# thrill/thrill

Measured on AMD Instinct MI355X. Metric: TeraSort keys/sec (100-byte recs), higher is better.
Workload: dtype u8; 1 GPU; terasort_10GiB_100B; records=107374182, record_bytes=100, seed=0x7421, parallelism=dp1

## Files before the change

thrill_amd/csrc/t9_sort_msb9.hip:

```cpp

#include "t9_common.h"
#include "t9_rank_scatter.h"

#include <cstdlib>
#include <vector>

#define T9_MSB_TILE 8192
#define NDIG9 512

__device__ inline u32 bucket_of9(const u32* s_abase, u32 pos) {
    u32 lo = 0, hi = 255;
    while (lo < hi) {
        u32 mid = (lo + hi + 1) >> 1;
        if (s_abase[mid] <= pos) lo = mid; else hi = mid - 1;
    }
    return lo;
}

__global__ __launch_bounds__(256) void k_hist_seg9(
    const u64* __restrict__ keys, const u32* __restrict__ abase,
    const u32* __restrict__ bucket_n, u32* __restrict__ hist) {
    __shared__ u32 s_cnt[NDIG9];
    __shared__ u32 s_abase[257];
    const u32 tid = threadIdx.x;
    s_abase[tid] = abase[tid];
    if (tid == 0) s_abase[256] = abase[256];
    s_cnt[tid] = 0;
    s_cnt[tid + 256] = 0;
    __syncthreads();
    const u64 tbase64 = (u64)blockIdx.x * T9_MSB_TILE;
    if (tbase64 < s_abase[256]) {
        const u32 tbase = (u32)tbase64;
        const u32 b = bucket_of9(s_abase, tbase);
        const u32 off = tbase - s_abase[b];
        const u32 tn = (bucket_n[b] > off)
                           ? ((bucket_n[b] - off < T9_MSB_TILE)
                                  ? bucket_n[b] - off
                                  : T9_MSB_TILE)
                           : 0;
        const u32 lane = tid & 63;
        for (u32 i0 = 0; i0 < (u32)T9_MSB_TILE; i0 += 256) {
            const u32 i = i0 + tid;
            const bool valid = i < tn;
            const u32 d =
                valid ? (u32)(keys[tbase + i] >> 47) & 511u : 0;
            t9_hist_ballot_add<9>(s_cnt, d, valid, lane);
        }
    }
    __syncthreads();
    hist[(u64)blockIdx.x * NDIG9 + tid] = s_cnt[tid];
    hist[(u64)blockIdx.x * NDIG9 + tid + 256] = s_cnt[tid + 256];
}

__global__ __launch_bounds__(256) void k_seg_scan9(
    u32* __restrict__ hist, const u32* __restrict__ abase,
    const u32* __restrict__ bucket_n, const u32* __restrict__ true_base,
    u32* __restrict__ sub_start, u32* __restrict__ sub_n) {
    const u32 b = blockIdx.x;
    const u32 tid = threadIdx.x;
    const u32 r0 = abase[b] / T9_MSB_TILE;
    const u32 rows = (bucket_n[b] + T9_MSB_TILE - 1) / T9_MSB_TILE;
    u32 tot0 = 0, tot1 = 0;
    for (u32 r = 0; r < rows; ++r) {
        tot0 += hist[(u64)(r0 + r) * NDIG9 + tid];
        tot1 += hist[(u64)(r0 + r) * NDIG9 + tid + 256];
    }
    __shared__ u32 sh[NDIG9];
    sh[tid] = tot0;
    sh[tid + 256] = tot1;
    __syncthreads();
    t9_scan_onewave<NDIG9>(sh, tid);
    __syncthreads();
    const u32 gstart0 = true_base[b] + sh[tid];
    const u32 gstart1 = true_base[b] + sh[tid + 256];
    sub_start[(u64)b * NDIG9 + tid] = gstart0;
    sub_start[(u64)b * NDIG9 + tid + 256] = gstart1;
    sub_n[(u64)b * NDIG9 + tid] = tot0;
    sub_n[(u64)b * NDIG9 + tid + 256] = tot1;
    u32 run0 = gstart0, run1 = gstart1;
    for (u32 r = 0; r < rows; ++r) {
        u32 v0 = hist[(u64)(r0 + r) * NDIG9 + tid];
        u32 v1 = hist[(u64)(r0 + r) * NDIG9 + tid + 256];
        hist[(u64)(r0 + r) * NDIG9 + tid] = run0;
        hist[(u64)(r0 + r) * NDIG9 + tid + 256] = run1;
        run0 += v0;
        run1 += v1;
    }
}

template <bool HAS_VAL>
__global__ __launch_bounds__(1024, 4) void k_scatter_seg9(
    const u64* __restrict__ in_keys, const u32* __restrict__ in_vals,
    const u32* __restrict__ abase, const u32* __restrict__ bucket_n,
    u64* __restrict__ out_keys, u32* __restrict__ out_vals,
    const u32* __restrict__ offs) {
    constexpr int TILE = T9_MSB_TILE;
    constexpr int NW = 16;
    constexpr int SUB = TILE / NW;
    constexpr int GROUPS = SUB / 64;
    __shared__ u64 s_okeys[TILE];
    __shared__ u32 s_ovals[HAS_VAL ? TILE : 1];
    __shared__ u16 s_rank[TILE];
    __shared__ u16 s_wcnt[NW * NDIG9];
    __shared__ u16 s_woff[NW * NDIG9];
    __shared__ u32 s_start[NDIG9];
    __shared__ u32 s_goff[NDIG9];
    __shared__ u32 s_abase[257];

    const u32 tid = threadIdx.x, wave = tid >> 6, lane = tid & 63;
    if (tid < 257) s_abase[tid] = abase[tid];
    __syncthreads();
    const u64 tbase64 = (u64)blockIdx.x * TILE;
    if (tbase64 >= s_abase[256]) return;
    const u32 tbase = (u32)tbase64;
    const u32 b = bucket_of9(s_abase, tbase);
    const u32 off_in_bucket = tbase - s_abase[b];
    const u32 bn = bucket_n[b];
    const u32 tn = (bn > off_in_bucket)
                       ? ((bn - off_in_bucket < (u32)TILE)
                              ? bn - off_in_bucket
                              : (u32)TILE)
                       : 0;

    if (tid < NDIG9)
        s_goff[tid] = offs[(u64)blockIdx.x * NDIG9 + tid];
    for (u32 t = lane; t < NDIG9; t += 64) s_wcnt[wave * NDIG9 + t] = 0;

    const u32 wbase = wave * SUB;
    for (int g = 0; g < GROUPS; ++g) {
        const u32 i = wbase + g * 64 + lane;
        const bool valid = i < tn;
        u32 d = 0;
        if (valid) d = (u32)(in_keys[tbase + i] >> 47) & 511u;
        u64 m = __ballot(valid);
        for (int bit = 0; bit < 9; ++bit) {
            u64 bb = __ballot((d >> bit) & 1u);
            m &= ((d >> bit) & 1u) ? bb : ~bb;
        }
        const u32 wr = (u32)__popcll(m & ((1ull << lane) - 1ull));
        const u32 before = valid ? (u32)s_wcnt[wave * NDIG9 + d] : 0;
        if (valid) {
            s_rank[i] = (u16)(before + wr);
            if (wr == 0)
                s_wcnt[wave * NDIG9 + d] =
                    (u16)(before + (u32)__popcll(m));
        }
    }
    __syncthreads();

    if (tid < NDIG9) {
        u32 run = 0;
        for (int w = 0; w < NW; ++w) {
            s_woff[w * NDIG9 + tid] = (u16)run;
            run += s_wcnt[w * NDIG9 + tid];
        }
        s_start[tid] = run;
    }
    __syncthreads();
    t9_scan_onewave<NDIG9>(s_start, tid);
    __syncthreads();

    for (int g = 0; g < GROUPS; ++g) {
        const u32 i = wbase + g * 64 + lane;
        if (i < tn) {
            const u64 k = in_keys[tbase + i];
            const u32 d = (u32)(k >> 47) & 511u;
            const u32 pos = s_start[d] + (u32)s_woff[wave * NDIG9 + d] +
                            s_rank[i];
            s_okeys[pos] = k;
            if (HAS_VAL) s_ovals[pos] = in_vals[tbase + i];
        }
    }
    __syncthreads();

    constexpr int CHUNKS = TILE / 1024;
    for (int c = 0; c < CHUNKS; ++c) {
        const u32 j = c * 1024 + tid;
        if (j < tn) {
            const u32 d = (u32)(s_okeys[j] >> 47) & 511u;
            const u64 gpos = (u64)s_goff[d] + (j - s_start[d]);
            out_keys[gpos] = s_okeys[j];
            if (HAS_VAL) out_vals[gpos] = s_ovals[j];
        }
    }
}

extern "C" {

void t9i_launch_hist_seg9(u32 grid, void* stream, const u64* keys,
                          const u32* abase, const u32* bucket_n,
                          u32* hist) {
    hipLaunchKernelGGL(k_hist_seg9, dim3(grid), dim3(256), 0,
                       (hipStream_t)stream, keys, abase, bucket_n, hist);
}

void t9i_launch_seg_scan9(u32 grid, void* stream, u32* hist,
                          const u32* abase, const u32* bucket_n,
                          const u32* true_base, u32* sub_start,
                          u32* sub_n) {
    hipLaunchKernelGGL(k_seg_scan9, dim3(grid), dim3(256), 0,
                       (hipStream_t)stream, hist, abase, bucket_n,
                       true_base, sub_start, sub_n);
}

void t9i_launch_scatter_seg9(u32 grid, int has_val, void* stream,
                             const u64* in_keys, const u32* in_vals,
                             const u32* abase, const u32* bucket_n,
                             u64* out_keys, u32* out_vals,
                             const u32* offs) {
    if (has_val)
        hipLaunchKernelGGL((k_scatter_seg9<true>), dim3(grid), dim3(1024),
                           0, (hipStream_t)stream, in_keys, in_vals, abase,
                           bucket_n, out_keys, out_vals, offs);
    else
        hipLaunchKernelGGL((k_scatter_seg9<false>), dim3(grid), dim3(1024),
                           0, (hipStream_t)stream, in_keys, in_vals, abase,
                           bucket_n, out_keys, out_vals, offs);
}

}
```

Baseline: 8.578 billion keys/s.

## Restructure MSB scatter kernel to cut LDS use and keep keys in registers

Rewrites the segmented 9-bit MSB scatter kernel. Keys and values are held in registers instead of being reloaded. The key and value staging buffers share one LDS region, per-key ranks are packed into registers, and the bucket lookup uses wave ballots instead of a shared-memory binary search. The digit scan uses shuffles, and tile indices are remapped so contiguous tiles land on the same XCD. The launch-bounds hint is raised so more blocks fit per CU. The risks are higher register pressure, which could cause spills at the new occupancy target, and subtle correctness hazards from aliasing LDS buffers and from the unconditional key loads past tn.

```diff
diff --git a/thrill_amd/csrc/t9_sort_msb9.hip b/thrill_amd/csrc/t9_sort_msb9.hip
--- a/thrill_amd/csrc/t9_sort_msb9.hip
+++ b/thrill_amd/csrc/t9_sort_msb9.hip
@@ -89,7 +89,7 @@
 }
 
 template <bool HAS_VAL>
-__global__ __launch_bounds__(1024, 4) void k_scatter_seg9(
+__global__ __launch_bounds__(1024, 8) void k_scatter_seg9(
     const u64* __restrict__ in_keys, const u32* __restrict__ in_vals,
     const u32* __restrict__ abase, const u32* __restrict__ bucket_n,
     u64* __restrict__ out_keys, u32* __restrict__ out_vals,
@@ -98,90 +98,162 @@
     constexpr int NW = 16;
     constexpr int SUB = TILE / NW;
     constexpr int GROUPS = SUB / 64;
-    __shared__ u64 s_okeys[TILE];
-    __shared__ u32 s_ovals[HAS_VAL ? TILE : 1];
-    __shared__ u16 s_rank[TILE];
-    __shared__ u16 s_wcnt[NW * NDIG9];
-    __shared__ u16 s_woff[NW * NDIG9];
-    __shared__ u32 s_start[NDIG9];
-    __shared__ u32 s_goff[NDIG9];
-    __shared__ u32 s_abase[257];
+    __shared__ __align__(16) u8 s_raw[TILE * 8];
+    u64* const s_okeys = (u64*)s_raw;
+    u32* const s_ovals = (u32*)s_raw;
+    static_assert(SUB <= 65535 && TILE <= 65535, "u16 counts and offsets");
+    static_assert(NW * 64 == 1024 && NDIG9 == 8 * 64,
+                  "one thread per key column, waves 0..7 own the digits");
+    __shared__ __align__(16) u16 s_wcnt[NW * NDIG9];
+    u32* const s_wtot = (u32*)s_raw;
+    u32* const s_delta = (u32*)s_wcnt;
 
     const u32 tid = threadIdx.x, wave = tid >> 6, lane = tid & 63;
-    if (tid < 257) s_abase[tid] = abase[tid];
-    __syncthreads();
-    const u64 tbase64 = (u64)blockIdx.x * TILE;
-    if (tbase64 >= s_abase[256]) return;
+    const u32 xper = gridDim.x >> 3, xrem = gridDim.x & 7;
+    const u32 xcd = blockIdx.x & 7;
+    const u32 tile = xcd * xper + (xcd < xrem ? xcd : xrem) +
+                     (blockIdx.x >> 3);
+    const u64 tbase64 = (u64)tile * TILE;
+    if (tbase64 >= abase[256]) return;
     const u32 tbase = (u32)tbase64;
-    const u32 b = bucket_of9(s_abase, tbase);
-    const u32 off_in_bucket = tbase - s_abase[b];
-    const u32 bn = bucket_n[b];
+
+    const u32 wbase = wave * SUB;
+    u64 key[GROUPS];
+#pragma unroll
+    for (int g = 0; g < GROUPS; ++g)
+        key[g] = in_keys[tbase + wbase + g * 64 + lane];
+    u32 ab[4], bnq[4];
+#pragma unroll
+    for (int q = 0; q < 4; ++q) {
+        ab[q] = abase[q * 64 + lane];
+        bnq[q] = bucket_n[q * 64 + lane];
+    }
+    u16* const wc = s_wcnt + wave * NDIG9;
+    for (u32 t = lane; t < NDIG9; t += 64) wc[t] = 0;
+
+    u32 nle = 0;
+#pragma unroll
+    for (int q = 0; q < 4; ++q)
+        nle += (u32)__popcll(__ballot(ab[q] <= tbase));
+    const u32 b = nle - 1, bq = b >> 6;
+    const u32 ab_b = (u32)__builtin_amdgcn_readlane(
+        (int)(bq == 0 ? ab[0] : bq == 1 ? ab[1] : bq == 2 ? ab[2] : ab[3]),
+        (int)(b & 63));
+    const u32 bn = (u32)__builtin_amdgcn_readlane(
+        (int)(bq == 0 ? bnq[0] : bq == 1 ? bnq[1] : bq == 2 ? bnq[2]
+                                                            : bnq[3]),
+        (int)(b & 63));
+    const u32 off_in_bucket = tbase - ab_b;
     const u32 tn = (bn > off_in_bucket)
                        ? ((bn - off_in_bucket < (u32)TILE)
                               ? bn - off_in_bucket
                               : (u32)TILE)
                        : 0;
-
-    if (tid < NDIG9)
-        s_goff[tid] = offs[(u64)blockIdx.x * NDIG9 + tid];
-    for (u32 t = lane; t < NDIG9; t += 64) s_wcnt[wave * NDIG9 + t] = 0;
-
-    const u32 wbase = wave * SUB;
+    if (tn == 0) return;
+
+    u32 pos2[GROUPS / 2] = {};
+#pragma unroll
     for (int g = 0; g < GROUPS; ++g) {
         const u32 i = wbase + g * 64 + lane;
         const bool valid = i < tn;
-        u32 d = 0;
-        if (valid) d = (u32)(in_keys[tbase + i] >> 47) & 511u;
-        u64 m = __ballot(valid);
+        const u32 d = (u32)(key[g] >> 47) & 511u;
+        u32 dlo = 0, dhi = 0;
+#pragma unroll
         for (int bit = 0; bit < 9; ++bit) {
-            u64 bb = __ballot((d >> bit) & 1u);
-            m &= ((d >> bit) & 1u) ? bb : ~bb;
-        }
+            const u32 own = 0u - ((d >> bit) & 1u);
+            const u64 bb = __ballot(own != 0);
+            dlo |= (u32)bb ^ own;
+            dhi |= (u32)(bb >> 32) ^ own;
+        }
+        const u64 m = __ballot(valid) & ~(((u64)dhi << 32) | dlo);
         const u32 wr = (u32)__popcll(m & ((1ull << lane) - 1ull));
-        const u32 before = valid ? (u32)s_wcnt[wave * NDIG9 + d] : 0;
-        if (valid) {
-            s_rank[i] = (u16)(before + wr);
-            if (wr == 0)
-                s_wcnt[wave * NDIG9 + d] =
-                    (u16)(before + (u32)__popcll(m));
-        }
-    }
-    __syncthreads();
-
+        const u32 before = wc[d];
+        pos2[g >> 1] |= (before + wr) << (16 * (g & 1));
+        if (valid && wr == 0) wc[d] = (u16)(before + (u32)__popcll(m));
+    }
+    u32 goff = 0;
+    if (tid < NDIG9) goff = offs[(u64)tile * NDIG9 + tid];
+    __syncthreads();
+
+    u32 excl = 0;
     if (tid < NDIG9) {
         u32 run = 0;
         for (int w = 0; w < NW; ++w) {
-            s_woff[w * NDIG9 + tid] = (u16)run;
-            run += s_wcnt[w * NDIG9 + tid];
-        }
-        s_start[tid] = run;
-    }
-    __syncthreads();
-    t9_scan_onewave<NDIG9>(s_start, tid);
-    __syncthreads();
-
+            const u32 c = s_wcnt[w * NDIG9 + tid];
+            s_wcnt[w * NDIG9 + tid] = (u16)run;
+            run += c;
+        }
+        u32 v = run;
+        for (int off = 1; off < 64; off <<= 1) {
+            const u32 y = __shfl_up(v, off);
+            if (lane >= (u32)off) v += y;
+        }
+        excl = v - run;
+        if (lane == 63) s_wtot[wave] = v;
+    }
+    __syncthreads();
+    u32 delta = 0;
+    if (tid < NDIG9) {
+        u32 start = excl;
+        for (u32 w = 0; w < wave; ++w) start += s_wtot[w];
+        for (int w = 0; w < NW; ++w)
+            s_wcnt[w * NDIG9 + tid] += (u16)start;
+        delta = goff - start;
+    }
+    __syncthreads();
+
+    u32 val[HAS_VAL ? GROUPS : 1];
+    if constexpr (HAS_VAL) {
+#pragma unroll
+        for (int g = 0; g < GROUPS; ++g)
+            val[g] = in_vals[tbase + wbase + g * 64 + lane];
+    }
+
+#pragma unroll
     for (int g = 0; g < GROUPS; ++g) {
         const u32 i = wbase + g * 64 + lane;
-        if (i < tn) {
-            const u64 k = in_keys[tbase + i];
-            const u32 d = (u32)(k >> 47) & 511u;
-            const u32 pos = s_start[d] + (u32)s_woff[wave * NDIG9 + d] +
-                            s_rank[i];
-            s_okeys[pos] = k;
-            if (HAS_VAL) s_ovals[pos] = in_vals[tbase + i];
-        }
-    }
-    __syncthreads();
-
-    constexpr int CHUNKS = TILE / 1024;
-    for (int c = 0; c < CHUNKS; ++c) {
-        const u32 j = c * 1024 + tid;
-        if (j < tn) {
-            const u32 d = (u32)(s_okeys[j] >> 47) & 511u;
-            const u64 gpos = (u64)s_goff[d] + (j - s_start[d]);
-            out_keys[gpos] = s_okeys[j];
-            if (HAS_VAL) out_vals[gpos] = s_ovals[j];
-        }
+        const u32 d = (u32)(key[g] >> 47) & 511u;
+        const u32 pos = ((pos2[g >> 1] >> (16 * (g & 1))) & 0xffffu) +
+                        (u32)wc[d];
+        if (i < tn) s_okeys[pos] = key[g];
+        pos2[g >> 1] += (u32)wc[d] << (16 * (g & 1));
+    }
+    __syncthreads();
+    if (tid < NDIG9) s_delta[tid] = delta;
+    __syncthreads();
+
+    u64 k[GROUPS];
+    u32 gpos[GROUPS];
+#pragma unroll
+    for (int c = 0; c < GROUPS; ++c) k[c] = s_okeys[c * 1024 + tid];
+#pragma unroll
+    for (int c = 0; c < GROUPS; ++c)
+        gpos[c] = s_delta[(u32)(k[c] >> 47) & 511u] + (c * 1024 + tid);
+    if constexpr (HAS_VAL) {
+        __syncthreads();
+#pragma unroll
+        for (int g = 0; g < GROUPS; ++g)
+            asm volatile("" : "+v"(val[g]));
+#pragma unroll
+        for (int g = 0; g < GROUPS; ++g) {
+            const u32 i = wbase + g * 64 + lane;
+            if (i < tn)
+                s_ovals[(pos2[g >> 1] >> (16 * (g & 1))) & 0xffffu] = val[g];
+        }
+        __builtin_amdgcn_sched_barrier(0);
+    }
+#pragma unroll
+    for (int c = 0; c < GROUPS; ++c)
+        if (c * 1024 + tid < tn) out_keys[gpos[c]] = k[c];
+    if (!HAS_VAL) return;
+    __syncthreads();
+    {
+        u32 v[GROUPS];
+#pragma unroll
+        for (int c = 0; c < GROUPS; ++c) v[c] = s_ovals[c * 1024 + tid];
+#pragma unroll
+        for (int c = 0; c < GROUPS; ++c)
+            if (c * 1024 + tid < tn) out_vals[gpos[c]] = v[c];
     }
 }
 
```

Result: faster. 9.068 billion keys/s (median of 6 runs) (+5.7%).
